# hyye/lio-mapping

Measured on AMD Instinct MI355X. Metric: sliding-window solves/sec, 64-line 130k-pt scans, window=15 (opt_window=5), higher is better.
Workload: dtype f64 (solve) / f32 (features); 1 GPU; HDL-64E outdoor_test_config_64, S_outdoor ray-cast scans, window_size=15 opt_window_size=5, one SolveOptimization per step, clouds resident in HBM; n_lidar_residuals=78236, local_map_points=76752, surf_stack_points=19386, parallelism=1 window

## Files before the change

### include/lio_c.h

```cpp
#ifndef LIO_C_H_
#define LIO_C_H_

#include <stddef.h>
#include <stdint.h>

#ifdef __cplusplus
extern "C" {
#endif

#define LIO_OK 0
#define LIO_ERR_ARG (-1)
#define LIO_ERR_STATE (-2)
#define LIO_ERR_DEVICE (-3)
#define LIO_ERR_CAPACITY (-4)

typedef struct {
  float q[4];
  float p[3];
} lio_transform_f;

const char *lio_backend(void);

typedef struct {
  double scan_period;
// ... 153 lines not shown
  int point_distance_factor;
  int prior_factor;
  int marginalization_factor;
  int enable_deskew;
  int cutoff_deskew;
  int keep_features;
  double acc_n, gyr_n, acc_w, gyr_w, g_norm;
  int max_num_iterations;
  double max_solver_time;
  int extrinsic_stage;
  int init_window_factor;
  int device_solve;
  int inline_marg;
  int stream_sync;
  int resident_moments;
} lio_est_config;

typedef struct {
  int iterations;
  int successful_steps;
  int termination;
  int n_lidar_residuals;
  int n_local_map;
  int laser_odom_iterations;
  int turn_off;
  int convergence_flag;
  int marginalized;
  double cost_pim_before, cost_ppp_before, cost_marg_before;
  double initial_cost, final_cost;
  double cost_trace[32];
// ... 100 lines not shown
```

### lio-mapping_amd/csrc/capi.hip

```cpp
#include <cstring>
#include <new>

#include "../../include/lio_c.h"
#include "../../include/lio_test_hooks.h"
#include "../../include/lio_ext.h"
#include "../../include/lio_full_cloud.h"
#include "../../include/lio_odom_batch.h"
#include "../../include/lio_frontend_batch.h"
#include "../../include/lio_map_batch.h"
#include "est_batch.h"
#include "seg_sort.h"
#include "estimator.h"
#include "rccl_comm.h"
#include "host_init.h"
#include "kf_batch.h"
#include <mutex>
#include <thread>
#include <atomic>
#include <algorithm>

#include "mapping.h"
#include "odometry.h"
#include "pointproc.h"

// ... 560 lines not shown
struct Scratch {
  hipStream_t s = nullptr;
  DBuf<float4> a, b, c;
  VoxelGridDev vox;
  KnnGrid grid;
  DBuf<uint8_t> valid;
  DBuf<float4> coef, abs_coef;
  DBuf<float> score, tf;
  DBuf<int32_t> idx;
  DBuf<float> sqd, nbr;
  DBuf<float> bounds;
  DBuf<double> gn_partials, gn_sums;
  DBuf<OdomState> gn_state;
  DBuf<KfDesc> gn_kd;
  DBuf<float> gn_rows;
};
static Scratch &scratch() {
  static thread_local Scratch sc;
  if (!sc.s) {
    int nd = 0;
    LIO_HIP(hipGetDeviceCount(&nd));
    if (nd <= 0) throw DeviceError("no HIP device: the product has no CPU path");
    LIO_HIP(hipStreamCreate(&sc.s));
  }
  return sc;
}

int lio_voxel_grid(const float *xyzi, size_t n, float leaf, float *out, size_t *n_out) {
  if ((!xyzi && n) || !out || !n_out || !(leaf > 0)) return LIO_ERR_ARG;
  return guarded([&] {
// ... 218 lines not shown
    host_cloud_bounds(map, n_map, mn, mx);
    sc.grid.build(sc.a.p, n_map, mn, mx, knn_cell_edge(mm), sc.s);
    FeatArgs fa{};
    fa.nframes = 1; fa.max_M = M; fa.min_match_sq_dis = mm; fa.min_plane_dis = mp;
    fa.fr[0].stack = sc.b.p; fa.fr[0].M = M; fa.fr[0].slot_off = 0; fa.fr[0].tf_index = 0;
    launch_odom_round(fa, 0, 0, 0, sc.gn_state.p, sc.grid.sorted(), sc.grid.cells(), sc.grid.desc(), sc.valid.p, sc.coef.p, sc.score.p, sc.gn_partials.p, sc.s,
                      nullptr, HostSignal(), lpq);
    if (nb) LIO_HIP(hipMemcpyAsync(partials_out, sc.gn_partials.p, size_t(nb) * 28 * sizeof(double), hipMemcpyDeviceToHost, sc.s));
    LIO_HIP(hipMemcpyAsync(state_out, sc.gn_state.p, sizeof(OdomState), hipMemcpyDeviceToHost, sc.s));
    LIO_HIP(hipStreamSynchronize(sc.s));
    *nb_out = nb;
    return LIO_OK;
  });
}

int lio_calculate_features(const float *map, size_t n_map, const float *stack, size_t m, const lio_transform_f *T, float mm, float mp,
                           uint8_t *valid, float *coeff, float *score) {
  if ((!map && n_map) || (!stack && m) || !T || !valid || !coeff || !score || !(mm > 0)) return LIO_ERR_ARG;
  return guarded([&] {
    Scratch &sc = scratch();
    sc.a.reserve(std::max<size_t>(n_map, 1)); sc.b.reserve(std::max<size_t>(m, 1));
    sc.valid.reserve(std::max<size_t>(m, 1)); sc.coef.reserve(std::max<size_t>(m, 1)); sc.score.reserve(std::max<size_t>(m, 1)); sc.tf.reserve(8);
    if (n_map) LIO_HIP(hipMemcpyAsync(sc.a.p, map, n_map * sizeof(float4), hipMemcpyHostToDevice, sc.s));
    if (m) LIO_HIP(hipMemcpyAsync(sc.b.p, stack, m * sizeof(float4), hipMemcpyHostToDevice, sc.s));
    float tf[8] = {T->q[0], T->q[1], T->q[2], T->q[3], T->p[0], T->p[1], T->p[2], 0.f};
    LIO_HIP(hipMemcpyAsync(sc.tf.p, tf, sizeof(tf), hipMemcpyHostToDevice, sc.s));
    float mn[3], mx[3];
    host_cloud_bounds(map, n_map, mn, mx);
    sc.grid.build(sc.a.p, n_map, mn, mx, knn_cell_edge(mm), sc.s);
    FeatArgs fa{};
// ... 87 lines not shown
  if (!h) return nullptr;
  EstConfig &e = h->cfg;
  e.W = c->window_size; e.Wo = c->opt_window_size;
  e.corner_filter_size = c->corner_filter_size; e.surf_filter_size = c->surf_filter_size;
  e.min_match_sq_dis = c->min_match_sq_dis; e.min_plane_dis = c->min_plane_dis;
  e.transform_lb = toT(c->transform_lb);
  e.opt_extrinsic = c->opt_extrinsic; e.imu_factor = c->imu_factor; e.point_distance_factor = c->point_distance_factor;
  e.prior_factor = c->prior_factor; e.marginalization_factor = c->marginalization_factor;
  e.enable_deskew = c->enable_deskew; e.cutoff_deskew = c->cutoff_deskew; e.keep_features = c->keep_features;
  e.pim.acc_n = c->acc_n; e.pim.gyr_n = c->gyr_n; e.pim.acc_w = c->acc_w; e.pim.gyr_w = c->gyr_w; e.pim.g_norm = c->g_norm;
  e.max_num_iterations = c->max_num_iterations; e.max_solver_time = c->max_solver_time; e.extrinsic_stage = c->extrinsic_stage;
  e.init_window_factor = c->init_window_factor > 0 ? c->init_window_factor : 1;
  e.device_solve = c->device_solve != 0; e.inline_marg = c->inline_marg != 0;
  e.stream_sync = c->stream_sync != 0;
  e.resident_moments = (c->resident_moments >= 1 && c->resident_moments <= 3) ? c->resident_moments : 0;
  h->map_cfg.corner_filter_size = c->corner_filter_size; h->map_cfg.surf_filter_size = c->surf_filter_size;
  h->map_cfg.min_match_sq_dis = c->min_match_sq_dis; h->map_cfg.min_plane_dis = c->min_plane_dis; h->map_cfg.num_max_iterations = 10;
  h->map_cfg.map_builder = 0; h->map_cfg.enable_4d = 1; h->map_cfg.skip_count = 2;
  int rc = guarded([&] {
    h->e.reset(new Estimator(e));
    if (e.device_solve) {
      h->solo.reset(new EstimatorBatch({h->e.get()}));
      EstimatorBatch *b = h->solo.get();
      h->e->solve_hook_ = [b](lio_solve_report *rep) { b->Solve(rep); return b->window_ok(0); };
    }
    return LIO_OK;
  });
  if (rc != LIO_OK) { delete h; return nullptr; }
  return h;
}
// ... 599 lines not shown
```

### lio-mapping_amd/csrc/cloud_device.h

```cpp
#pragma once
#include <hip/hip_runtime.h>

#include <cfloat>
#include <climits>

#include "cloud_kernels.h"
#include "hmath.h"

#if defined(__HIPCC__)
namespace lio {

__device__ inline bool finite3(const float4 &p) { return isfinite(p.x) && isfinite(p.y) && isfinite(p.z); }
__device__ inline bool finite3(const Vec3<float> &p) { return isfinite(p.x) && isfinite(p.y) && isfinite(p.z); }


template <bool NORMALISE_CONJ>
__device__ __forceinline__ float4 to_end_point(float4 p, float s, const Quat<float> &qe, const Vec3<float> &te) {
  p.x -= s * te.x; p.y -= s * te.y; p.z -= s * te.z;
  Quat<float> qid;
  Quat<float> qs = slerp(qid, s, qe, FLT_EPSILON);
  Quat<float> qc = conj(qs);
  if (NORMALISE_CONJ) qc = normalized(qc);
  Vec3<float> v = rotate(qc, Vec3<float>(p.x, p.y, p.z));
  v = rotate(qe, v);
// ... 206 lines not shown
template <int K>
__device__ __forceinline__ void knn_insert(unsigned long long key, int j, unsigned long long (&bk)[K], int (&bj)[K]) {
  if (key < bk[K - 1]) {
    bk[K - 1] = key; bj[K - 1] = j;
#pragma unroll
    for (int k = K - 1; k > 0; --k) {
      const bool sw = bk[k - 1] > bk[k];
      const unsigned long long tk = sw ? bk[k - 1] : bk[k];
      const int tj = sw ? bj[k - 1] : bj[k];
      bk[k - 1] = sw ? bk[k] : bk[k - 1];
      bj[k - 1] = sw ? bj[k] : bj[k - 1];
      bk[k] = tk; bj[k] = tj;
    }
  }
}
template <int K, int LPQ>
__device__ inline void knn_scan_group(const Vec3<float> &q, bool active, int sub, const float4 *__restrict__ map,
                                      const int *__restrict__ cells, const GridDesc &g, float (&bd)[K], int (&bi)[K], int (&bj)[K]) {
  unsigned long long bk[K];
#pragma unroll
  for (int k = 0; k < K; ++k) { bk[k] = knn_key(INFINITY, INT_MAX); bj[k] = 0; }
  int cx, cy, cz;
  cell_of(q.x, q.y, q.z, g, cx, cy, cz);
  if (!finite3(q) || cx < 0 || cy < 0 || cz < 0 || cx >= g.dims[0] || cy >= g.dims[1] || cz >= g.dims[2]) active = false;
  if (active) {
    const int x0 = max(cx - 1, 0), x1 = min(cx + 1, g.dims[0] - 1);
    if constexpr (LPQ <= 2) {
      const float uy = q.y * g.inv_cell, uz = q.z * g.inv_cell;
      const float fy = uy - floorf(uy), fz = uz - floorf(uz);
      const float cell = 1.0f / g.inv_cell;
      const float ey_lo = fmaxf(fy - 1e-3f, 0.f) * cell, ey_hi = fmaxf(1.0f - fy - 1e-3f, 0.f) * cell;
      const float ez_lo = fmaxf(fz - 1e-3f, 0.f) * cell, ez_hi = fmaxf(1.0f - fz - 1e-3f, 0.f) * cell;
      auto walk = [&](int j) {
// ... 27 lines not shown
          if (qq == 1) { s1 = a; c2 = c1 + len; }
          if (qq == 2) { s2 = a; c3 = c2 + len; }
          if (qq == 3) { s3 = a; T = c3 + len; }
        }
        for (int f = 0; f < T; ++f) {
          int j = s0 + f * LPQ;
          j = f >= c1 ? s1 + (f - c1) * LPQ : j;
          j = f >= c2 ? s2 + (f - c2) * LPQ : j;
          j = f >= c3 ? s3 + (f - c3) * LPQ : j;
          walk(j);
        }
      }
    } else {
      int rs[9], pre[10];
      pre[0] = 0;
#pragma unroll
      for (int r = 0; r < 9; ++r) {
        const int z = cz + r / 3 - 1, y = cy + r % 3 - 1;
        const bool in = z >= 0 && z < g.dims[2] && y >= 0 && y < g.dims[1];
        const int row = g.dims[0] * (y + g.dims[1] * z);
        const int a = in ? cells[row + x0] : 0, b = in ? cells[row + x1 + 1] : 0;
        rs[r] = a;
        pre[r + 1] = b - a;
      }
#pragma unroll
      for (int r = 0; r < 9; ++r) pre[r + 1] = pre[r] + max(pre[r + 1], 0);
      const int T = pre[9];
      for (int base = sub; base < T; base += LPQ * KNN_BATCH) {
        float4 p[KNN_BATCH];
        int jj[KNN_BATCH];
#pragma unroll
        for (int b = 0; b < KNN_BATCH; ++b) {
          const int f = base + b * LPQ;
          int j = f + rs[0];
#pragma unroll
          for (int r = 1; r < 9; ++r) j = f >= pre[r] ? f - pre[r] + rs[r] : j;
          jj[b] = f < T ? j : -1;
          p[b] = f < T ? map[j] : make_float4(0, 0, 0, 0);
        }
#pragma unroll
        for (int b = 0; b < KNN_BATCH; ++b) {
          if (jj[b] < 0) continue;
          float ddx = p[b].x - q.x, ddy = p[b].y - q.y, ddz = p[b].z - q.z;
          float d = ddx * ddx;
          d += ddy * ddy;
          d += ddz * ddz;
          knn_insert<K>(knn_key(d, __float_as_int(p[b].w)), jj[b], bk, bj);
        }
      }
    }
  }
#pragma unroll
  for (int m = 1; m < LPQ; m <<= 1) {
    unsigned long long ok[K]; int oj[K];
#pragma unroll
    for (int k = 0; k < K; ++k) {
      const unsigned int lo = __shfl_xor(static_cast<unsigned int>(bk[k]), m, 64), hi = __shfl_xor(static_cast<unsigned int>(bk[k] >> 32), m, 64);
      ok[k] = (static_cast<unsigned long long>(hi) << 32) | lo;
      oj[k] = __shfl_xor(bj[k], m, 64);
    }
#pragma unroll
    for (int c = 0; c < K; ++c) knn_insert<K>(ok[c], oj[c], bk, bj);
  }
#pragma unroll
  for (int k = 0; k < K; ++k) { bd[k] = __uint_as_float(static_cast<unsigned int>(bk[k] >> 32)); bi[k] = int(static_cast<unsigned int>(bk[k])); }
}

struct FeatScalars { float min_match_sq_dis, min_plane_dis; int mapping_mode; float fixed_pz[3]; };
__device__ __forceinline__ FeatScalars feat_scalars(const FeatArgs &a) {
  return FeatScalars{a.min_match_sq_dis, a.min_plane_dis, a.mapping_mode, {a.fixed_pz[0], a.fixed_pz[1], a.fixed_pz[2]}};
}
struct FeatResult { bool owner; uint8_t ok; float4 c; float sc; float4 abs; float4 po; int slot; };
template <bool MAPPING>
__device__ __forceinline__ FeatResult features_fit(const FeatScalars &a, int slot, const Quat<float> &q, const Vec3<float> &t, const float4 &po,
                                                   const Vec3<float> &sel, float bd4, int bi4, const int (&bj)[5], const float4 *__restrict__ map) {
  FeatResult res;
  res.owner = true; res.ok = 0; res.c = make_float4(0, 0, 0, 0); res.sc = 0; res.abs = make_float4(0, 0, 0, 0); res.po = po; res.slot = slot;
  uint8_t ok = 0;
  float4 c = make_float4(0, 0, 0, 0);
  float sc = 0;
// ... 184 lines not shown
  if (!isfinite(t.x)) t.x = 0;
  if (!isfinite(t.y)) t.y = 0;
  if (!isfinite(t.z)) t.z = 0;
  st->T[0] = q.x; st->T[1] = q.y; st->T[2] = q.z; st->T[3] = q.w; st->T[4] = t.x; st->T[5] = t.y; st->T[6] = t.z;
  Quat<float> d = R0 * conj(q);
  float ang = 2.f * atan2f(norm(d.vec()), fabsf(d.w));
  float delta_r = float(double(ang) * 180.0 / M_PI);
  double dt0 = double(X[3] * 100), dt1 = double(X[4] * 100), dt2 = double(X[5] * 100);
  float delta_t = float(sqrt(dt0 * dt0 + dt1 * dt1 + dt2 * dt2));
  st->iters = iter + 1;
  if (double(delta_r) < 0.05 && double(delta_t) < 0.05) st->converged = 1;
}


#define ODOM_ROUND_THREADS 256
template <int LPQ, int THREADS = ODOM_ROUND_THREADS>
__device__ __forceinline__ double odom_round_block(const FeatScalars fs, FeatFrame fr, const Quat<float> q, const Vec3<float> t, const float4 *__restrict__ map,
                                                   const int *__restrict__ cells, const GridDesc &g, uint8_t *__restrict__ valid, float4 *__restrict__ coef,
                                                   float *__restrict__ score, int base_slot, int round, int keep, int block) {
  constexpr int QPB = THREADS / LPQ;
  static_assert(QPB <= 64, "the fit phase is one wave");
  __shared__ int s_bj[QPB][5];
  __shared__ float s_bd4[QPB];
  __shared__ int s_bi4[QPB];
  const int M = fr.M;
  fr.slot_off = base_slot + (keep ? round * M : 0);
  {
    const int ql = threadIdx.x / LPQ, sub = threadIdx.x % LPQ;
    const int i = block * QPB + ql;
    const bool active = i < M;
    const float4 po = active ? fr.stack[i] : make_float4(0, 0, 0, 0);
    const Vec3<float> r = rotate(q, Vec3<float>(po.x, po.y, po.z));
    const Vec3<float> sel(r.x + t.x, r.y + t.y, r.z + t.z);
    float bd[5]; int bi[5], bj[5];
    knn_scan_group<5, LPQ>(sel, active, sub, map, cells, g, bd, bi, bj);
    if (sub == 0) {
#pragma unroll
      for (int k = 0; k < 5; ++k) s_bj[ql][k] = bj[k];
      s_bd4[ql] = bd[4]; s_bi4[ql] = bi[4];
    }
  }
  __syncthreads();
  double v = 0;
  if (threadIdx.x < 64) {
    const int ql = threadIdx.x;
    double acc[28];
#pragma unroll
    for (int k = 0; k < 28; ++k) acc[k] = 0;
    const int i = block * QPB + ql;
    if (ql < QPB && i < M) {
      const float4 po = fr.stack[i];
      const Vec3<float> r = rotate(q, Vec3<float>(po.x, po.y, po.z));
      const Vec3<float> sel(r.x + t.x, r.y + t.y, r.z + t.z);
      int bj[5];
// ... 81 lines not shown
```

### lio-mapping_amd/csrc/cloud_kernels.h

```cpp
#pragma once
#include <cmath>
#include <cstdint>

#include "dev.h"
#include "hmath.h"

namespace lio {

struct VoxParams {
  float mn[3], mx[3];
  int minb[3], divb[3];
  int overflow;
  int n_valid;
};

struct Affine3f { float m[12]; };

#define LIO_MAX_FRAMES 32

struct ConcatSeg { const float4 *src; int n; int dst_off; int set_intensity; float intensity; Affine3f tf; int identity; };
struct ConcatArgs { ConcatSeg seg[LIO_MAX_FRAMES]; int nseg; int total; };
void launch_transform_concat(const ConcatArgs &a, float4 *dst, hipStream_t s);

void launch_deskew_to_end(float4 *pts, int n, const float q[4], const float p[3], float time_factor, hipStream_t s, bool keep_intensity = false);
// ... 115 lines not shown
  int kz;
  int nsel;
};
inline OdomState odom_state_at(const Rigid<float> &T) {
  OdomState st{};
  st.T[0] = T.rot.x; st.T[1] = T.rot.y; st.T[2] = T.rot.z; st.T[3] = T.rot.w;
  st.T[4] = T.pos.x; st.T[5] = T.pos.y; st.T[6] = T.pos.z;
  return st;
}
inline void point_on_z_axis(const Rigid<float> &T, float pz[3]) {
  const Vec3<float> z = rotate(T.rot, Vec3<float>(0.f, 0.f, 10.f));
  pz[0] = z.x + T.pos.x; pz[1] = z.y + T.pos.y; pz[2] = z.z + T.pos.z;
}
int odom_rows_blocks(int nslots);
int odom_round_blocks(int M, int lpq);
void launch_odom_round(const FeatArgs &a, int base_slot, int round, int keep, OdomState *st, const float4 *map_sorted, const int *cells, const GridDesc &g,
                       uint8_t *valid, float4 *coef, float *score, double *partials, hipStream_t s, OdomState *mail = nullptr,
                       const HostSignal &sig = HostSignal(), int lpq = 8);

void launch_gn_rows_map(const float4 *stack, int m, const uint8_t *valid, const float4 *coef, const OdomState *st, int b_from_coef, uint8_t *ok_out,
                        float *rows_out, hipStream_t s);
void launch_gn_fold(const double *partials, int nblocks, int wide, double *sums_out, hipStream_t s);
void launch_gn_step(const double *sums, OdomState *st, int iter, int min_rows, int left_update, hipStream_t s);

struct KfDesc {
  int slot_off, Mc, Ms;
  int map;
  int nb;
  int part_off;
  float pz[3];
};
struct KfMapDesc {
  const float4 *corner_sorted; const int *corner_cells; GridDesc corner_grid;
// ... 34 lines not shown
```

### lio-mapping_amd/csrc/cloud_kernels.hip

```cpp
#include <cstring>
#include <hip/hip_runtime.h>
#include <rocprim/rocprim.hpp>

#include <cfloat>
#include <climits>

#include "cloud_kernels.h"
#include "cloud_device.h"

namespace lio {

__global__ void k_transform_concat(ConcatArgs a, float4 *__restrict__ dst) {
  int gid = blockIdx.x * blockDim.x + threadIdx.x;
  if (gid >= a.total) return;
  int sidx = 0;
  for (int k = 1; k < a.nseg; ++k)
    if (gid >= a.seg[k].dst_off) sidx = k;
  const ConcatSeg &sg = a.seg[sidx];
  int local = gid - sg.dst_off;
  float4 p = sg.src[local];
  float4 o;
  if (sg.identity) {
    o = p;
  } else {
// ... 487 lines not shown
  __syncthreads();
  if (threadIdx.x < 28) {
    double v = 0;
    for (int w = 0; w < ODOM_ROW_THREADS / 64; ++w) v += sm[w][threadIdx.x];
    partials[block_x * 28 + threadIdx.x] = v;
  }
}

__device__ __forceinline__ void odom_update_body(const double *__restrict__ partials, int nblocks, OdomState *st, int iter, int min_rows,
                                                 int left_update) {
  __shared__ double ssum[28];
  reduce_partials28(partials, nblocks, ssum);
  odom_update_from_sums(ssum, st, iter, min_rows, left_update);
}

template <int LPQ>
__global__ void __launch_bounds__(ODOM_ROUND_THREADS) k_odom_round(FeatArgs a, const OdomState *__restrict__ st, const float4 *__restrict__ map,
                                                                  const int *__restrict__ cells, GridDesc g, uint8_t *__restrict__ valid,
                                                                  float4 *__restrict__ coef, float *__restrict__ score, double *__restrict__ partials,
                                                                  int base_slot, int round, int keep) {
  if (st->converged) return;
  const float *tp = st->T;
  const Quat<float> q(tp[3], tp[0], tp[1], tp[2]);
  const Vec3<float> t(tp[4], tp[5], tp[6]);
  const double v = odom_round_block<LPQ>(feat_scalars(a), a.fr[0], q, t, map, cells, g, valid, coef, score, base_slot, round, keep, int(blockIdx.x));
  if (threadIdx.x < 28) partials[size_t(blockIdx.x) * 28 + threadIdx.x] = v;
}

__global__ void __launch_bounds__(1024) k_odom_update_wide(const double *__restrict__ partials, int nblocks, OdomState *st, int iter, int min_rows,
                                                           int left_update, OdomState *mail, HostSignal sig) {
  odom_update_wide_block(partials, nblocks, st, iter, min_rows, left_update, mail, sig);
}
__global__ void __launch_bounds__(256) k_solve_setup(SolveSetup a, float *__restrict__ d_transforms, OdomState *__restrict__ d_odom, uint8_t *__restrict__ valid,
                                                     size_t n_valid) {
  clear_valid_block(valid, n_valid);
  if (blockIdx.x == 0) {
    for (int k = threadIdx.x; k < a.ntf * 8; k += 256) d_transforms[k] = a.tf[k >> 3][k & 7];
    if (a.set_odom) odom_state_init(d_odom, a.odom_T, false);
  }
}
void launch_solve_setup(const SolveSetup &a, float *d_transforms, OdomState *d_odom, uint8_t *valid, size_t n_valid, hipStream_t s) {
  const int nb = std::max(1, cdiv((long long)n_valid, 256 * 16));
  hipLaunchKernelGGL(k_solve_setup, dim3(nb), dim3(256), 0, s, a, d_transforms, d_odom, valid, n_valid);
  LIO_HIP(hipGetLastError());
}

int odom_round_blocks(int M, int lpq) { return std::max(1, cdiv((long long)M * lpq, ODOM_ROUND_THREADS)); }
void launch_odom_round(const FeatArgs &a, int base_slot, int round, int keep, OdomState *st, const float4 *map_sorted, const int *cells, const GridDesc &g,
                       uint8_t *valid, float4 *coef, float *score, double *partials, hipStream_t s, OdomState *mail, const HostSignal &sig, int lpq) {
  const int M = a.fr[0].M;
  if (M <= 0) return;
  const int nb = odom_round_blocks(M, lpq);
  if (lpq == 4)
    hipLaunchKernelGGL(k_odom_round<4>, dim3(nb), dim3(ODOM_ROUND_THREADS), 0, s, a, st, map_sorted, cells, g, valid, coef, score, partials, base_slot, round, keep);
  else
    hipLaunchKernelGGL(k_odom_round<8>, dim3(nb), dim3(ODOM_ROUND_THREADS), 0, s, a, st, map_sorted, cells, g, valid, coef, score, partials, base_slot, round, keep);
  hipLaunchKernelGGL(k_odom_update_wide, dim3(1), dim3(1024), 0, s, partials, nb, st, round, 0, 0, mail, sig);
  LIO_HIP(hipGetLastError());
}

__global__ void __launch_bounds__(256) k_gn_rows_map(const float4 *__restrict__ stack, int m, const uint8_t *__restrict__ valid, const float4 *__restrict__ coef,
                                                     const OdomState *__restrict__ st, int b_from_coef, uint8_t *__restrict__ ok_out,
                                                     float *__restrict__ rows_out) {
  const int i = blockIdx.x * blockDim.x + threadIdx.x;
  if (i >= m) return;
  Quat<float> q(st->T[3], st->T[0], st->T[1], st->T[2]);
  Vec3<float> t(st->T[4], st->T[5], st->T[6]);
  Mat3<float> Rm = toRot(q);
  Mat3<float> Rinv = toRot(qinverse(q));
  float a[6] = {0, 0, 0, 0, 0, 0}, bb = 0;
  const bool ok = valid[i] != 0;
  if (ok) odom_row_form(stack[i], coef[i], q, t, Rm, Rinv, b_from_coef, a, bb);
// ... 147 lines not shown
```

### lio-mapping_amd/csrc/estimator.h

```cpp
#pragma once
#include <climits>
#include <condition_variable>
#include <exception>
#include <functional>
#include <memory>
#include <mutex>
#include <thread>
#include <vector>

#include "../../include/lio_c.h"
#include "cloud_kernels.h"
#include "host_init.h"
#include "host_solver.h"
#include "batch_kernels.h"
#include "resident_moments.h"
#include "solve_step.h"

namespace lio {

typedef Rigid<float> Rigidf;
typedef Rigid<double> Rigidd;

struct EstConfig {
  int W = 15, Wo = 5;
  float corner_filter_size = 0.2f, surf_filter_size = 0.4f, min_match_sq_dis = 1.0f, min_plane_dis = 0.2f;
  Rigidf transform_lb;
  bool opt_extrinsic = false, imu_factor = true, point_distance_factor = false, prior_factor = false, marginalization_factor = true,
       enable_deskew = true, cutoff_deskew = false, keep_features = false;
  PimNoise pim;
  int max_num_iterations = 10;
  double max_solver_time = 0.10;
  int extrinsic_stage = 2;
  int init_window_factor = 3;
  bool device_solve = false, inline_marg = false, stream_sync = false;
  int resident_moments = 0;
};

struct DeviceCloud {
  DBuf<float4> buf;
  size_t n = 0;
  uint64_t id = 0;
  DeviceCloud() = default;
  DeviceCloud(DeviceCloud &&o) noexcept : buf(std::move(o.buf)), n(o.n), id(o.id) { o.n = 0; o.id = 0; }
  DeviceCloud &operator=(DeviceCloud &&o) noexcept {
    if (this != &o) { buf = std::move(o.buf); n = o.n; id = o.id; o.n = 0; o.id = 0; }
    return *this;
  }
};

struct StampedPose { double time; Rigidf T; };
// ... 249 lines not shown
  std::vector<size_t> size_surf_stack_;
  std::vector<StampedPose> imu_stamped_;
  DeviceCloud local_, local_filtered_, scratch_cloud_, upload_;
  VoxelGridDev vox_;
  KnnGrid grid_;
  DBuf<uint8_t> f_valid_;
  DBuf<float4> f_coef_;
  DBuf<float> f_score_;
  std::vector<int> slot_off_, nslots_;
  size_t total_slots_ = 0;
  EstimatorBatch *feat_batch_ = nullptr;
  int feat_batch_w_ = -1;
  DBuf<float> d_transforms_;
  DBuf<OdomState> d_odom_;
  DBuf<double> d_odom_partials_, d_moment_partials_, d_moment_out_;
  HostBuf<double> h_moment_out_;
  HostBuf<OdomState> h_odom_;
  HostBuf<unsigned> h_signal_;
  unsigned signal_seq_[2] = {0, 0};
  bool host_signal_ = true;
  int device_id_ = 0;
  HostSignal moment_signal_{};
  bool frames_dirty_ = true;
  std::unique_ptr<HostState> snap_;
  std::vector<DeviceCloud> snap_stacks_;
  bool map_refresh_ = false;
  std::vector<OptSlot> opt_ring_;
  long frame_seq_ = 0;
  std::shared_ptr<DeviceCloud> corner_last_;
  std::vector<std::shared_ptr<DeviceCloud>> corner_pool_;
// ... 16 lines not shown
```

### lio-mapping_amd/csrc/estimator.hip

```cpp
#include "estimator.h"
#include "est_batch.h"
#include "mapping.h"
#include "marg_kernels.h"
#include "rccl_comm.h"

#include <atomic>
#include <cfloat>
#include <climits>
#include <cstring>

namespace lio {

static const bool g_debug_timing = std::getenv("LIO_DEBUG_TIMING") != nullptr;

static V3d R2ypr(const M3d &R) {
  V3d n(R(0, 0), R(1, 0), R(2, 0)), o(R(0, 1), R(1, 1), R(2, 1)), a(R(0, 2), R(1, 2), R(2, 2));
  double y = atan2(n.y, n.x);
  double p = atan2(-n.z, n.x * cos(y) + n.y * sin(y));
  double r = atan2(a.x * sin(y) - a.y * cos(y), -o.x * sin(y) + o.y * cos(y));
  return V3d(y, p, r) / M_PI * 180.0;
}
static M3d ypr2R(const V3d &ypr) {
  double y = ypr.x / 180.0 * M_PI, p = ypr.y / 180.0 * M_PI, r = ypr.z / 180.0 * M_PI;
  M3d Rz, Ry, Rx;
// ... 632 lines not shown
    timers_.end(th, sf);
    if (sf != stream_) LIO_HIP(hipEventRecord(ev_join_, sf));
  }
  laser_odom_iters_ = 0; laser_odom_kz_ = 0;
  if (cfg_.imu_factor) {
    OdomState st{};
    bool have_state = false;
    std::memcpy(st.T, pl.tf[W_], 8 * sizeof(float));
    const int M = int(stacks_[W_].n);
    const bool mail = host_signal_ && !timers_.on;
    HostSignal sig{};
    if (M > 0) {
      const int lpq = 8;
      const int nb = odom_round_blocks(M, lpq);
      d_odom_partials_.reserve(size_t(nb) * 28);
      FeatArgs fo{};
      fo.min_match_sq_dis = cfg_.min_match_sq_dis; fo.min_plane_dis = cfg_.min_plane_dis;
      fo.nframes = 1; fo.max_M = M;
      fo.fr[0].stack = stacks_[W_].buf.p; fo.fr[0].M = M; fo.fr[0].tf_index = 0; fo.fr[0].slot_off = slot_off_[W_];
      const int chunk_end[4] = {3, 5, 7, 10};
      int chunk = 0;
      for (int iter = 0; iter < 10; ++iter) {
        if (iter == chunk_end[chunk]) {
          if (mail) {
            wait_host_signal(sig, stream_);
          } else {
            LIO_HIP(hipMemcpyAsync(h_odom_.p, d_odom_.p, sizeof(st), hipMemcpyDeviceToHost, stream_));
            LIO_HIP(hipStreamSynchronize(stream_));
          }
          st = *h_odom_.p;
          if (st.converged) { have_state = true; break; }
          ++chunk;
        }
        if (mail) { sig.flag = h_signal_.p + 128; sig.seq = ++signal_seq_[1]; }
        const double ns = keep_mult > 1 ? double(iter + 1) * M : double(M);
        int t1h = timers_.begin(KT_ODOM_FEATURES, 16.0 * (double(M) + double(local_filtered_.n)) + 72.0 * M + 33.0 * ns, stream_);
        launch_odom_round(fo, slot_off_[W_], iter, keep_mult > 1 ? 1 : 0, d_odom_.p, grid_.sorted(), grid_.cells(), grid_.desc(), f_valid_.p, f_coef_.p,
                          f_score_.p, d_odom_partials_.p, stream_, mail ? h_odom_.p : nullptr, sig, lpq);
        timers_.end(t1h, stream_);
      }
    }
    LIO_HIP(hipStreamWaitEvent(stream_, ev_join_, 0));
    if (!have_state) {
      if (sig.flag) {
        wait_host_signal(sig, stream_);
      } else {
        LIO_HIP(hipMemcpyAsync(h_odom_.p, d_odom_.p, sizeof(st), hipMemcpyDeviceToHost, stream_));
        LIO_HIP(hipStreamSynchronize(stream_));
      }
      st = *h_odom_.p;
      timers_.resolve();
    }
    ApplyOdomState(st);
// ... 544 lines not shown
```

### lio-mapping_amd/lio_amd/capi.py

```python
from __future__ import annotations

import ctypes as C
import os

import numpy as np

_HERE = os.path.dirname(os.path.abspath(__file__))
HIP_LIB_PATH = os.environ.get("LIO_HIP_LIB") or os.path.join(os.path.dirname(_HERE), "csrc", "liblio_hip.so")

c_double_p = C.POINTER(C.c_double)
c_float_p = C.POINTER(C.c_float)
c_int32_p = C.POINTER(C.c_int32)
c_uint8_p = C.POINTER(C.c_uint8)
c_uint16_p = C.POINTER(C.c_uint16)


class TransformF(C.Structure):
    _fields_ = [("q", C.c_float * 4), ("p", C.c_float * 3)]

    @staticmethod
    def make(q_xyzw, p):
        t = TransformF()
        for i in range(4):
            t.q[i] = float(q_xyzw[i])
# ... 51 lines not shown
        ("cutoff_deskew", C.c_int),
        ("keep_features", C.c_int),
        ("acc_n", C.c_double),
        ("gyr_n", C.c_double),
        ("acc_w", C.c_double),
        ("gyr_w", C.c_double),
        ("g_norm", C.c_double),
        ("max_num_iterations", C.c_int),
        ("max_solver_time", C.c_double),
        ("extrinsic_stage", C.c_int),
        ("init_window_factor", C.c_int),
        ("device_solve", C.c_int),
        ("inline_marg", C.c_int),
        ("stream_sync", C.c_int),
        ("resident_moments", C.c_int),
    ]


class SolveReport(C.Structure):
    _fields_ = [
        ("iterations", C.c_int),
        ("successful_steps", C.c_int),
        ("termination", C.c_int),
        ("n_lidar_residuals", C.c_int),
        ("n_local_map", C.c_int),
        ("laser_odom_iterations", C.c_int),
        ("turn_off", C.c_int),
        ("convergence_flag", C.c_int),
        ("marginalized", C.c_int),
        ("cost_pim_before", C.c_double),
# ... 162 lines not shown
    "lio_gn_fold": (C.c_int, [c_double_p, C.c_int, C.c_int, c_double_p]),
    "lio_gn_step": (C.c_int, [C.c_int, c_double_p, C.c_void_p, C.c_int, C.c_int, C.c_int, C.c_void_p]),
    "lio_gn_round": (C.c_int, [c_float_p, C.c_size_t, c_float_p, C.c_size_t, C.POINTER(TransformF), C.c_float, C.c_float, C.c_int, c_int32_p,
                               c_double_p, C.c_void_p]),
}
GN_STATE = np.dtype([("T", np.float32, 8), ("converged", np.int32), ("iters", np.int32), ("degenerate", np.int32), ("kz", np.int32),
                     ("nsel", np.int32)])
_EXT_SIGS = {
    "lio_est_map": (C.c_void_p, [C.c_void_p]),
    "lio_est_set_map_refresh": (C.c_int, [C.c_void_p, C.c_int]),
    "lio_est_refresh_map": (C.c_int, [C.c_void_p]),
    "lio_map_get_surround": (C.c_size_t, [C.c_void_p, C.c_float, c_float_p]),
    "lio_est_get_last_map_refresh": (C.c_int, [C.c_void_p, C.POINTER(C.c_int), C.POINTER(TransformF), C.POINTER(C.c_int), C.POINTER(C.c_uint32),
                                               C.POINTER(C.c_int), C.POINTER(C.c_size_t), c_float_p, C.POINTER(C.c_size_t), c_float_p]),
}
_FULL_SIGS = {
    "lio_odom_full_to_end": (C.c_int, [C.c_void_p, c_float_p, C.c_size_t, c_float_p]),
    "lio_map_set_full_cloud": (C.c_int, [C.c_void_p, c_float_p, C.c_size_t]),
    "lio_map_get_full_cloud": (C.c_size_t, [C.c_void_p, c_float_p]),
    "lio_est_set_full_cloud": (C.c_int, [C.c_void_p, C.c_int]),
    "lio_est_get_full_stack": (C.c_size_t, [C.c_void_p, C.c_int, c_float_p, C.POINTER(C.c_int)]),
    "lio_est_get_registered_full": (C.c_int, [C.c_void_p, C.c_int, C.POINTER(TransformF), C.POINTER(C.c_size_t), c_float_p]),
    "lio_est_get_full_transform_es": (C.c_int, [C.c_void_p, C.c_int, C.POINTER(TransformF)]),
    "lio_deskew_to_end": (C.c_int, [c_float_p, C.c_size_t, C.POINTER(TransformF), C.c_float, C.c_int, c_float_p]),
}
FULL_MAP_FRAME, FULL_SENSOR_RAW, FULL_SENSOR_END = 1, 2, 3
_c_float_pp, _c_size_p = C.POINTER(c_float_p), C.POINTER(C.c_size_t)
_ODOM_BATCH_SIGS = {
    "lio_odom_process_batch": (C.c_int, [C.POINTER(C.c_void_p), C.c_int, _c_float_pp, _c_size_p, _c_float_pp, _c_size_p, _c_float_pp, _c_size_p,
                                         _c_float_pp, _c_size_p, C.POINTER(TransformF), C.POINTER(TransformF), c_int32_p, c_int32_p]),
# ... 49 lines not shown
        for name, (res, args) in _TEST_SIGS.items():
            fn = getattr(self.dll, name, None)
            if fn is None:
                self.missing.append(name)
                continue
            fn.restype = res
            fn.argtypes = args
        self.backend = self.dll.lio_backend().decode()
        self.has_ext = self.backend.startswith("hip")
        if self.has_ext:
            for name, (res, args) in (list(_EXT_SIGS.items()) + list(_FULL_SIGS.items()) + list(_ODOM_BATCH_SIGS.items()) + list(_FRONTEND_SIGS.items())
                                      + list(_MAP_BATCH_SIGS.items())):
                fn = getattr(self.dll, name)
                fn.restype = res
                fn.argtypes = args

    def deskew_to_end(self, xyzi, T_es: TransformF, time_factor=10.0, keep_intensity=False):
        c = _f32(xyzi).reshape(-1, 4)
        out = np.zeros_like(c)
        _chk(self.dll.lio_deskew_to_end(_fp(c), c.shape[0], C.byref(T_es), time_factor, 1 if keep_intensity else 0, _fp(out)), "lio_deskew_to_end")
        return out

    @staticmethod
    def _laser_frames(transforms, pims):
        n = len(transforms)
        T = (TransformF * n)(*[TransformF.make(q, p) for q, p in transforms])
        P = (C.c_void_p * n)(*[(p.h if p is not None else None) for p in pims])
        return n, T, P

    def imu_estimate_extrinsic_rotation(self, transforms, pims, T_lb):
# ... 146 lines not shown
        _chk(self.dll.lio_gn_step(int(family), s_.ctypes.data_as(c_double_p), si.ctypes.data, int(iter), int(min_rows), int(left_update),
                                  so.ctypes.data), "lio_gn_step")
        return so[0]

    def gn_round(self, map_xyzi, stack_xyzi, T: TransformF, lanes_per_query, min_match_sq_dis=1.0, min_plane_dis=0.2):
        m_ = _f32(map_xyzi).reshape(-1, 4)
        s_ = _f32(stack_xyzi).reshape(-1, 4)
        m = s_.shape[0]
        nb = np.zeros(1, dtype=np.int32)
        partials = np.zeros((max(1, -(-m * int(lanes_per_query) // 256)), 28), dtype=np.float64)
        so = np.zeros(1, dtype=GN_STATE)
        _chk(self.dll.lio_gn_round(_fp(m_), m_.shape[0], _fp(s_), m, C.byref(T), float(min_match_sq_dis), float(min_plane_dis),
                                   int(lanes_per_query), nb.ctypes.data_as(c_int32_p), partials.ctypes.data_as(c_double_p), so.ctypes.data),
             "lio_gn_round")
        return partials[: int(nb[0])].copy(), so[0]

    def calculate_features(self, map_xyzi, stack_xyzi, T: TransformF, min_match_sq_dis=1.0, min_plane_dis=0.2):
        m_ = _f32(map_xyzi).reshape(-1, 4)
        s_ = _f32(stack_xyzi).reshape(-1, 4)
        valid = np.zeros(s_.shape[0], dtype=np.uint8)
        coeff = np.zeros((s_.shape[0], 4), dtype=np.float32)
        score = np.zeros(s_.shape[0], dtype=np.float32)
        _chk(
            self.dll.lio_calculate_features(
                _fp(m_), m_.shape[0], _fp(s_), s_.shape[0], C.byref(T), min_match_sq_dis, min_plane_dis, valid.ctypes.data_as(c_uint8_p), _fp(coeff), _fp(score)
            ),
            "lio_calculate_features",
        )
        return valid, coeff, score

# ... 824 lines not shown
```

Baseline: 2116 solves/s.

## Bound later-round KNN search with previous round's neighbour list

Odometry Gauss-Newton rounds now save each query's 5 nearest neighbours. Later rounds use those points' distances, under the new pose, as an upper bound on the search. The grid walk then skips neighbouring cell rows and x-extents that lie entirely beyond the bound, and skips heap inserts above it. This is on by default (round_search=0), and it adds per-query neighbour-list writes and reads plus some bound computation in exchange for less map-point scanning.

```diff
diff --git a/include/lio_c.h b/include/lio_c.h
--- a/include/lio_c.h
+++ b/include/lio_c.h
@@ -191,6 +191,7 @@
   int inline_marg;
   int stream_sync;
   int resident_moments;
+  int round_search;
 } lio_est_config;
 
 typedef struct {
diff --git a/include/lio_round_search.h b/include/lio_round_search.h
--- /dev/null
+++ b/include/lio_round_search.h
@@ -0,0 +1,17 @@
+#ifndef LIO_ROUND_SEARCH_H
+#define LIO_ROUND_SEARCH_H
+
+#include "lio_c.h"
+
+#ifdef __cplusplus
+extern "C" {
+#endif
+
+int lio_gn_rounds(const float *map_xyzi, size_t n_map, const float *stack_xyzi, size_t m, const lio_transform_f *T, int n_rounds,
+                  float min_match_sq_dis, float min_plane_dis, int lanes_per_query, int search, int32_t *nb_out, uint8_t *valid_out,
+                  float *coeff_out, double *partials_out, int32_t *idx_out, int32_t *n_bounded_out);
+
+#ifdef __cplusplus
+}
+#endif
+#endif
diff --git a/lio-mapping_amd/csrc/capi.hip b/lio-mapping_amd/csrc/capi.hip
--- a/lio-mapping_amd/csrc/capi.hip
+++ b/lio-mapping_amd/csrc/capi.hip
@@ -8,6 +8,7 @@
 #include "../../include/lio_odom_batch.h"
 #include "../../include/lio_frontend_batch.h"
 #include "../../include/lio_map_batch.h"
+#include "../../include/lio_round_search.h"
 #include "est_batch.h"
 #include "seg_sort.h"
 #include "estimator.h"
@@ -598,6 +599,7 @@
   DBuf<OdomState> gn_state;
   DBuf<KfDesc> gn_kd;
   DBuf<float> gn_rows;
+  DBuf<int> gn_nn, gn_idx, gn_count;
 };
 static Scratch &scratch() {
   static thread_local Scratch sc;
@@ -846,6 +848,49 @@
   });
 }
 
+int lio_gn_rounds(const float *map, size_t n_map, const float *stack, size_t m, const lio_transform_f *T, int n_rounds, float mm, float mp, int lpq,
+                  int search, int32_t *nb_out, uint8_t *valid_out, float *coeff_out, double *partials_out, int32_t *idx_out, int32_t *n_bounded_out) {
+  if ((!map && n_map) || !stack || !m || !T || !nb_out || !valid_out || !coeff_out || !partials_out || !idx_out || !n_bounded_out) return LIO_ERR_ARG;
+  if (!(lpq == 4 || lpq == 8) || !(search == 0 || search == 1) || n_rounds < 1 || n_rounds > 16) return LIO_ERR_ARG;
+  if (!(mm > 0) || !std::isfinite(mm) || !(mp > 0) || !std::isfinite(mp)) return LIO_ERR_ARG;
+  for (int r = 0; r < n_rounds; ++r)
+    if (!finite_T(T + r)) return LIO_ERR_ARG;
+  if (m > size_t(INT_MAX) / 8 || n_map > size_t(INT_MAX)) return LIO_ERR_CAPACITY;
+  return guarded([&] {
+    Scratch &sc = scratch();
+    const int M = int(m), nb = odom_round_blocks(M, lpq);
+    sc.a.reserve(std::max<size_t>(n_map, 1)); sc.b.reserve(m);
+    sc.valid.reserve(m); sc.coef.reserve(m); sc.score.reserve(m);
+    sc.gn_partials.reserve(size_t(nb) * 28); sc.gn_state.reserve(1);
+    sc.gn_nn.reserve(m * 5); sc.gn_idx.reserve(m * 5); sc.gn_count.reserve(1);
+    if (n_map) LIO_HIP(hipMemcpyAsync(sc.a.p, map, n_map * sizeof(float4), hipMemcpyHostToDevice, sc.s));
+    LIO_HIP(hipMemcpyAsync(sc.b.p, stack, m * sizeof(float4), hipMemcpyHostToDevice, sc.s));
+    float mn[3], mx[3];
+    host_cloud_bounds(map, n_map, mn, mx);
+    sc.grid.build(sc.a.p, n_map, mn, mx, knn_cell_edge(mm), sc.s);
+    FeatArgs fa{};
+    fa.nframes = 1; fa.max_M = M; fa.min_match_sq_dis = mm; fa.min_plane_dis = mp;
+    fa.fr[0].stack = sc.b.p; fa.fr[0].M = M; fa.fr[0].slot_off = 0; fa.fr[0].tf_index = 0;
+    RoundList rl;
+    rl.nn = search == 0 ? sc.gn_nn.p : nullptr; rl.idx_out = sc.gn_idx.p; rl.n_bounded = sc.gn_count.p;
+    for (int r = 0; r < n_rounds; ++r) {
+      const OdomState st = odom_state_at(toT(T[r]));
+      LIO_HIP(hipMemcpyAsync(sc.gn_state.p, &st, sizeof(st), hipMemcpyHostToDevice, sc.s));
+      LIO_HIP(hipMemsetAsync(sc.gn_count.p, 0, sizeof(int), sc.s));
+      launch_odom_round(fa, 0, r, 0, sc.gn_state.p, sc.grid.sorted(), sc.grid.cells(), sc.grid.desc(), sc.valid.p, sc.coef.p, sc.score.p, sc.gn_partials.p,
+                        sc.s, nullptr, HostSignal(), lpq, rl, search == 0 ? (r == 0 ? 1 : 2) : 0);
+      LIO_HIP(hipMemcpyAsync(valid_out + size_t(r) * m, sc.valid.p, m, hipMemcpyDeviceToHost, sc.s));
+      LIO_HIP(hipMemcpyAsync(coeff_out + size_t(r) * m * 4, sc.coef.p, m * sizeof(float4), hipMemcpyDeviceToHost, sc.s));
+      LIO_HIP(hipMemcpyAsync(partials_out + size_t(r) * nb * 28, sc.gn_partials.p, size_t(nb) * 28 * sizeof(double), hipMemcpyDeviceToHost, sc.s));
+      LIO_HIP(hipMemcpyAsync(idx_out + size_t(r) * m * 5, sc.gn_idx.p, m * 5 * sizeof(int), hipMemcpyDeviceToHost, sc.s));
+      LIO_HIP(hipMemcpyAsync(n_bounded_out + r, sc.gn_count.p, sizeof(int), hipMemcpyDeviceToHost, sc.s));
+      LIO_HIP(hipStreamSynchronize(sc.s));
+    }
+    *nb_out = nb;
+    return LIO_OK;
+  });
+}
+
 int lio_calculate_features(const float *map, size_t n_map, const float *stack, size_t m, const lio_transform_f *T, float mm, float mp,
                            uint8_t *valid, float *coeff, float *score) {
   if ((!map && n_map) || (!stack && m) || !T || !valid || !coeff || !score || !(mm > 0)) return LIO_ERR_ARG;
@@ -963,6 +1008,7 @@
   e.device_solve = c->device_solve != 0; e.inline_marg = c->inline_marg != 0;
   e.stream_sync = c->stream_sync != 0;
   e.resident_moments = (c->resident_moments >= 1 && c->resident_moments <= 3) ? c->resident_moments : 0;
+  e.round_search = c->round_search == 1 ? 1 : 0;
   h->map_cfg.corner_filter_size = c->corner_filter_size; h->map_cfg.surf_filter_size = c->surf_filter_size;
   h->map_cfg.min_match_sq_dis = c->min_match_sq_dis; h->map_cfg.min_plane_dis = c->min_plane_dis; h->map_cfg.num_max_iterations = 10;
   h->map_cfg.map_builder = 0; h->map_cfg.enable_4d = 1; h->map_cfg.skip_count = 2;
diff --git a/lio-mapping_amd/csrc/cloud_device.h b/lio-mapping_amd/csrc/cloud_device.h
--- a/lio-mapping_amd/csrc/cloud_device.h
+++ b/lio-mapping_amd/csrc/cloud_device.h
@@ -244,9 +244,11 @@
     }
   }
 }
-template <int K, int LPQ>
+template <int K, int LPQ, bool BOUND = false>
 __device__ inline void knn_scan_group(const Vec3<float> &q, bool active, int sub, const float4 *__restrict__ map,
-                                      const int *__restrict__ cells, const GridDesc &g, float (&bd)[K], int (&bi)[K], int (&bj)[K]) {
+                                      const int *__restrict__ cells, const GridDesc &g, float (&bd)[K], int (&bi)[K], int (&bj)[K],
+                                      unsigned long long B = 0) {
+  static_assert(!BOUND || LPQ > 2, "the bounded walk is the multi-lane form");
   unsigned long long bk[K];
 #pragma unroll
   for (int k = 0; k < K; ++k) { bk[k] = knn_key(INFINITY, INT_MAX); bj[k] = 0; }
@@ -304,12 +306,30 @@
     } else {
       int rs[9], pre[10];
       pre[0] = 0;
+      float D = 0.f, ex_lo = 0.f, ex_hi = 0.f, ey_lo = 0.f, ey_hi = 0.f, ez_lo = 0.f, ez_hi = 0.f;
+      if constexpr (BOUND) {
+        D = __uint_as_float(static_cast<unsigned int>(B >> 32));
+        const float ux = q.x * g.inv_cell, uy = q.y * g.inv_cell, uz = q.z * g.inv_cell;
+        const float fx = ux - floorf(ux), fy = uy - floorf(uy), fz = uz - floorf(uz);
+        const float cell = 1.0f / g.inv_cell;
+        ex_lo = fmaxf(fx - 1e-3f, 0.f) * cell; ex_hi = fmaxf(1.0f - fx - 1e-3f, 0.f) * cell;
+        ey_lo = fmaxf(fy - 1e-3f, 0.f) * cell; ey_hi = fmaxf(1.0f - fy - 1e-3f, 0.f) * cell;
+        ez_lo = fmaxf(fz - 1e-3f, 0.f) * cell; ez_hi = fmaxf(1.0f - fz - 1e-3f, 0.f) * cell;
+      }
 #pragma unroll
       for (int r = 0; r < 9; ++r) {
         const int z = cz + r / 3 - 1, y = cy + r % 3 - 1;
-        const bool in = z >= 0 && z < g.dims[2] && y >= 0 && y < g.dims[1];
+        bool in = z >= 0 && z < g.dims[2] && y >= 0 && y < g.dims[1];
         const int row = g.dims[0] * (y + g.dims[1] * z);
-        const int a = in ? cells[row + x0] : 0, b = in ? cells[row + x1 + 1] : 0;
+        int xa = x0, xb = x1;
+        if constexpr (BOUND) {
+          const float ey = r % 3 == 0 ? ey_lo : (r % 3 == 2 ? ey_hi : 0.f), ez = r / 3 == 0 ? ez_lo : (r / 3 == 2 ? ez_hi : 0.f);
+          const float e2 = ey * ey + ez * ez;
+          in = in && !(e2 > D);
+          xa = ex_lo * ex_lo + e2 > D ? cx : x0;
+          xb = ex_hi * ex_hi + e2 > D ? cx : x1;
+        }
+        const int a = in ? cells[row + xa] : 0, b = in ? cells[row + xb + 1] : 0;
         rs[r] = a;
         pre[r + 1] = b - a;
       }
@@ -335,7 +355,12 @@
           float d = ddx * ddx;
           d += ddy * ddy;
           d += ddz * ddz;
-          knn_insert<K>(knn_key(d, __float_as_int(p[b].w)), jj[b], bk, bj);
+          const unsigned long long key = knn_key(d, __float_as_int(p[b].w));
+          if constexpr (BOUND) {
+            if (key <= B) knn_insert<K>(key, jj[b], bk, bj);
+          } else {
+            knn_insert<K>(key, jj[b], bk, bj);
+          }
         }
       }
     }
@@ -354,6 +379,44 @@
   }
 #pragma unroll
   for (int k = 0; k < K; ++k) { bd[k] = __uint_as_float(static_cast<unsigned int>(bk[k] >> 32)); bi[k] = int(static_cast<unsigned int>(bk[k])); }
+}
+
+template <int LPQ>
+__device__ __forceinline__ unsigned long long knn_prev_bound(const Vec3<float> &q, bool active, int sub, const int *prev,
+                                                             const float4 *__restrict__ map, const GridDesc &g, bool &bounded) {
+  constexpr unsigned long long BROKEN = ~0ull;
+  int cx, cy, cz;
+  const bool inside = cell_of(q.x, q.y, q.z, g, cx, cy, cz);
+  const bool ok = active && finite3(q) && inside && prev[4] >= 0;
+  unsigned long long key = 0;
+#pragma unroll
+  for (int kk = 0; kk < (5 + LPQ - 1) / LPQ; ++kk) {
+    const int k = sub + kk * LPQ;
+    if (ok && k < 5) {
+      const int j = prev[k];
+      unsigned long long kj = BROKEN;
+      if (unsigned(j) < unsigned(g.n_points)) {
+        const float4 pc = map[j];
+        int px, py, pz;
+        cell_of(pc.x, pc.y, pc.z, g, px, py, pz);
+        px = min(max(px, 0), g.dims[0] - 1); py = min(max(py, 0), g.dims[1] - 1); pz = min(max(pz, 0), g.dims[2] - 1);
+        float ddx = pc.x - q.x, ddy = pc.y - q.y, ddz = pc.z - q.z;
+        float d = ddx * ddx;
+        d += ddy * ddy;
+        d += ddz * ddz;
+        if (abs(px - cx) <= 1 && abs(py - cy) <= 1 && abs(pz - cz) <= 1) kj = knn_key(d, __float_as_int(pc.w));
+      }
+      key = kj > key ? kj : key;
+    }
+  }
+#pragma unroll
+  for (int m = 1; m < LPQ; m <<= 1) {
+    const unsigned int lo = __shfl_xor(static_cast<unsigned int>(key), m, 64), hi = __shfl_xor(static_cast<unsigned int>(key >> 32), m, 64);
+    const unsigned long long o = (static_cast<unsigned long long>(hi) << 32) | lo;
+    key = o > key ? o : key;
+  }
+  bounded = ok && key != BROKEN;
+  return bounded ? key : knn_key(INFINITY, INT_MAX);
 }
 
 struct FeatScalars { float min_match_sq_dis, min_plane_dis; int mapping_mode; float fixed_pz[3]; };
@@ -568,10 +631,11 @@
 
 
 #define ODOM_ROUND_THREADS 256
-template <int LPQ, int THREADS = ODOM_ROUND_THREADS>
+template <int LPQ, int THREADS = ODOM_ROUND_THREADS, int LIST = 0, bool STATS = false>
 __device__ __forceinline__ double odom_round_block(const FeatScalars fs, FeatFrame fr, const Quat<float> q, const Vec3<float> t, const float4 *__restrict__ map,
                                                    const int *__restrict__ cells, const GridDesc &g, uint8_t *__restrict__ valid, float4 *__restrict__ coef,
-                                                   float *__restrict__ score, int base_slot, int round, int keep, int block) {
+                                                   float *__restrict__ score, int base_slot, int round, int keep, int block,
+                                                   const RoundList rl = RoundList()) {
   constexpr int QPB = THREADS / LPQ;
   static_assert(QPB <= 64, "the fit phase is one wave");
   __shared__ int s_bj[QPB][5];
@@ -587,11 +651,29 @@
     const Vec3<float> r = rotate(q, Vec3<float>(po.x, po.y, po.z));
     const Vec3<float> sel(r.x + t.x, r.y + t.y, r.z + t.z);
     float bd[5]; int bi[5], bj[5];
-    knn_scan_group<5, LPQ>(sel, active, sub, map, cells, g, bd, bi, bj);
+    if constexpr (LIST == 2) {
+      bool bounded;
+      const unsigned long long B = knn_prev_bound<LPQ>(sel, active, sub, rl.nn + size_t(i) * 5, map, g, bounded);
+      if constexpr (STATS)
+        if (bounded && sub == 0) atomicAdd(rl.n_bounded, 1);
+      knn_scan_group<5, LPQ, true>(sel, active, sub, map, cells, g, bd, bi, bj, B);
+    } else {
+      knn_scan_group<5, LPQ>(sel, active, sub, map, cells, g, bd, bi, bj);
+    }
     if (sub == 0) {
 #pragma unroll
       for (int k = 0; k < 5; ++k) s_bj[ql][k] = bj[k];
       s_bd4[ql] = bd[4]; s_bi4[ql] = bi[4];
+      if constexpr (LIST != 0)
+        if (active) {
+#pragma unroll
+          for (int k = 0; k < 5; ++k) rl.nn[size_t(i) * 5 + k] = (k == 4 && bi[4] == INT_MAX) ? -1 : bj[k];
+        }
+      if constexpr (STATS)
+        if (active) {
+#pragma unroll
+          for (int k = 0; k < 5; ++k) rl.idx_out[size_t(i) * 5 + k] = bi[k];
+        }
     }
   }
   __syncthreads();
diff --git a/lio-mapping_amd/csrc/cloud_kernels.h b/lio-mapping_amd/csrc/cloud_kernels.h
--- a/lio-mapping_amd/csrc/cloud_kernels.h
+++ b/lio-mapping_amd/csrc/cloud_kernels.h
@@ -153,9 +153,10 @@
 }
 int odom_rows_blocks(int nslots);
 int odom_round_blocks(int M, int lpq);
+struct RoundList { int *nn = nullptr; int *idx_out = nullptr; int *n_bounded = nullptr; };
 void launch_odom_round(const FeatArgs &a, int base_slot, int round, int keep, OdomState *st, const float4 *map_sorted, const int *cells, const GridDesc &g,
                        uint8_t *valid, float4 *coef, float *score, double *partials, hipStream_t s, OdomState *mail = nullptr,
-                       const HostSignal &sig = HostSignal(), int lpq = 8);
+                       const HostSignal &sig = HostSignal(), int lpq = 8, const RoundList &rl = RoundList(), int list_mode = 0);
 
 void launch_gn_rows_map(const float4 *stack, int m, const uint8_t *valid, const float4 *coef, const OdomState *st, int b_from_coef, uint8_t *ok_out,
                         float *rows_out, hipStream_t s);
diff --git a/lio-mapping_amd/csrc/cloud_kernels.hip b/lio-mapping_amd/csrc/cloud_kernels.hip
--- a/lio-mapping_amd/csrc/cloud_kernels.hip
+++ b/lio-mapping_amd/csrc/cloud_kernels.hip
@@ -1,4 +1,5 @@
 #include <cstring>
+#include <stdexcept>
 #include <hip/hip_runtime.h>
 #include <rocprim/rocprim.hpp>
 
@@ -525,16 +526,17 @@
   odom_update_from_sums(ssum, st, iter, min_rows, left_update);
 }
 
-template <int LPQ>
+template <int LPQ, int LIST = 0, bool STATS = false>
 __global__ void __launch_bounds__(ODOM_ROUND_THREADS) k_odom_round(FeatArgs a, const OdomState *__restrict__ st, const float4 *__restrict__ map,
                                                                   const int *__restrict__ cells, GridDesc g, uint8_t *__restrict__ valid,
                                                                   float4 *__restrict__ coef, float *__restrict__ score, double *__restrict__ partials,
-                                                                  int base_slot, int round, int keep) {
+                                                                  int base_slot, int round, int keep, RoundList rl) {
   if (st->converged) return;
   const float *tp = st->T;
   const Quat<float> q(tp[3], tp[0], tp[1], tp[2]);
   const Vec3<float> t(tp[4], tp[5], tp[6]);
-  const double v = odom_round_block<LPQ>(feat_scalars(a), a.fr[0], q, t, map, cells, g, valid, coef, score, base_slot, round, keep, int(blockIdx.x));
+  const double v = odom_round_block<LPQ, ODOM_ROUND_THREADS, LIST, STATS>(feat_scalars(a), a.fr[0], q, t, map, cells, g, valid, coef, score, base_slot, round,
+                                                                        keep, int(blockIdx.x), rl);
   if (threadIdx.x < 28) partials[size_t(blockIdx.x) * 28 + threadIdx.x] = v;
 }
 
@@ -557,16 +559,26 @@
 }
 
 int odom_round_blocks(int M, int lpq) { return std::max(1, cdiv((long long)M * lpq, ODOM_ROUND_THREADS)); }
+using OdomRoundKernel = void (*)(FeatArgs, const OdomState *, const float4 *, const int *, GridDesc, uint8_t *, float4 *, float *, double *, int, int, int,
+                                 RoundList);
+template <int LPQ, bool STATS>
+static OdomRoundKernel odom_round_kernel(int list_mode) {
+  return list_mode == 0 ? k_odom_round<LPQ, 0, STATS> : list_mode == 1 ? k_odom_round<LPQ, 1, STATS> : k_odom_round<LPQ, 2, STATS>;
+}
 void launch_odom_round(const FeatArgs &a, int base_slot, int round, int keep, OdomState *st, const float4 *map_sorted, const int *cells, const GridDesc &g,
-                       uint8_t *valid, float4 *coef, float *score, double *partials, hipStream_t s, OdomState *mail, const HostSignal &sig, int lpq) {
+                       uint8_t *valid, float4 *coef, float *score, double *partials, hipStream_t s, OdomState *mail, const HostSignal &sig, int lpq,
+                       const RoundList &rl, int list_mode) {
   const int M = a.fr[0].M;
   if (M <= 0) return;
   const int nb = odom_round_blocks(M, lpq);
-  if (lpq == 4)
-    hipLaunchKernelGGL(k_odom_round<4>, dim3(nb), dim3(ODOM_ROUND_THREADS), 0, s, a, st, map_sorted, cells, g, valid, coef, score, partials, base_slot, round, keep);
-  else
-    hipLaunchKernelGGL(k_odom_round<8>, dim3(nb), dim3(ODOM_ROUND_THREADS), 0, s, a, st, map_sorted, cells, g, valid, coef, score, partials, base_slot, round, keep);
-  hipLaunchKernelGGL(k_odom_update_wide, dim3(1), dim3(1024), 0, s, partials, nb, st, round, 0, 0, mail, sig);
+  const bool stats = rl.idx_out != nullptr;
+  if (list_mode < 0 || list_mode > 2 || (list_mode != 0 && !rl.nn) || (stats != (rl.n_bounded != nullptr)))
+    throw std::invalid_argument("launch_odom_round: neighbour list and mode do not agree");
+  const OdomRoundKernel k = stats ? (lpq == 4 ? odom_round_kernel<4, true>(list_mode) : odom_round_kernel<8, true>(list_mode))
+                                  : (lpq == 4 ? odom_round_kernel<4, false>(list_mode) : odom_round_kernel<8, false>(list_mode));
+  hipLaunchKernelGGL(k, dim3(nb), dim3(ODOM_ROUND_THREADS), 0, s, a, st, map_sorted, cells, g, valid, coef, score, partials, base_slot, round, keep, rl);
+  if (!stats)
+    hipLaunchKernelGGL(k_odom_update_wide, dim3(1), dim3(1024), 0, s, partials, nb, st, round, 0, 0, mail, sig);
   LIO_HIP(hipGetLastError());
 }
 
diff --git a/lio-mapping_amd/csrc/estimator.h b/lio-mapping_amd/csrc/estimator.h
--- a/lio-mapping_amd/csrc/estimator.h
+++ b/lio-mapping_amd/csrc/estimator.h
@@ -34,6 +34,7 @@
   int init_window_factor = 3;
   bool device_solve = false, inline_marg = false, stream_sync = false;
   int resident_moments = 0;
+  int round_search = 0;
 };
 
 struct DeviceCloud {
@@ -313,6 +314,7 @@
   DBuf<float> d_transforms_;
   DBuf<OdomState> d_odom_;
   DBuf<double> d_odom_partials_, d_moment_partials_, d_moment_out_;
+  DBuf<int> d_odom_nn_;
   HostBuf<double> h_moment_out_;
   HostBuf<OdomState> h_odom_;
   HostBuf<unsigned> h_signal_;
diff --git a/lio-mapping_amd/csrc/estimator.hip b/lio-mapping_amd/csrc/estimator.hip
--- a/lio-mapping_amd/csrc/estimator.hip
+++ b/lio-mapping_amd/csrc/estimator.hip
@@ -670,6 +670,9 @@
       const int lpq = 8;
       const int nb = odom_round_blocks(M, lpq);
       d_odom_partials_.reserve(size_t(nb) * 28);
+      const bool bounded = cfg_.round_search == 0;
+      RoundList rl{};
+      if (bounded) { d_odom_nn_.reserve(size_t(M) * 5); rl.nn = d_odom_nn_.p; }
       FeatArgs fo{};
       fo.min_match_sq_dis = cfg_.min_match_sq_dis; fo.min_plane_dis = cfg_.min_plane_dis;
       fo.nframes = 1; fo.max_M = M;
@@ -692,7 +695,7 @@
         const double ns = keep_mult > 1 ? double(iter + 1) * M : double(M);
         int t1h = timers_.begin(KT_ODOM_FEATURES, 16.0 * (double(M) + double(local_filtered_.n)) + 72.0 * M + 33.0 * ns, stream_);
         launch_odom_round(fo, slot_off_[W_], iter, keep_mult > 1 ? 1 : 0, d_odom_.p, grid_.sorted(), grid_.cells(), grid_.desc(), f_valid_.p, f_coef_.p,
-                          f_score_.p, d_odom_partials_.p, stream_, mail ? h_odom_.p : nullptr, sig, lpq);
+                          f_score_.p, d_odom_partials_.p, stream_, mail ? h_odom_.p : nullptr, sig, lpq, rl, bounded ? (iter == 0 ? 1 : 2) : 0);
         timers_.end(t1h, stream_);
       }
     }
diff --git a/lio-mapping_amd/lio_amd/capi.py b/lio-mapping_amd/lio_amd/capi.py
--- a/lio-mapping_amd/lio_amd/capi.py
+++ b/lio-mapping_amd/lio_amd/capi.py
@@ -89,6 +89,7 @@
         ("inline_marg", C.c_int),
         ("stream_sync", C.c_int),
         ("resident_moments", C.c_int),
+        ("round_search", C.c_int),
     ]
 
 
@@ -281,6 +282,10 @@
     "lio_est_get_last_map_refresh": (C.c_int, [C.c_void_p, C.POINTER(C.c_int), C.POINTER(TransformF), C.POINTER(C.c_int), C.POINTER(C.c_uint32),
                                                C.POINTER(C.c_int), C.POINTER(C.c_size_t), c_float_p, C.POINTER(C.c_size_t), c_float_p]),
 }
+_ROUND_SEARCH_SIGS = {
+    "lio_gn_rounds": (C.c_int, [c_float_p, C.c_size_t, c_float_p, C.c_size_t, C.POINTER(TransformF), C.c_int, C.c_float, C.c_float, C.c_int, C.c_int,
+                                c_int32_p, c_uint8_p, c_float_p, c_double_p, c_int32_p, c_int32_p]),
+}
 _FULL_SIGS = {
     "lio_odom_full_to_end": (C.c_int, [C.c_void_p, c_float_p, C.c_size_t, c_float_p]),
     "lio_map_set_full_cloud": (C.c_int, [C.c_void_p, c_float_p, C.c_size_t]),
@@ -360,6 +365,11 @@
                 fn = getattr(self.dll, name)
                 fn.restype = res
                 fn.argtypes = args
+            for name, (res, args) in _ROUND_SEARCH_SIGS.items():
+                fn = getattr(self.dll, name, None)
+                if fn is not None:
+                    fn.restype = res
+                    fn.argtypes = args
 
     def deskew_to_end(self, xyzi, T_es: TransformF, time_factor=10.0, keep_intensity=False):
         c = _f32(xyzi).reshape(-1, 4)
@@ -536,6 +546,25 @@
                                    int(lanes_per_query), nb.ctypes.data_as(c_int32_p), partials.ctypes.data_as(c_double_p), so.ctypes.data),
              "lio_gn_round")
         return partials[: int(nb[0])].copy(), so[0]
+
+    def gn_rounds(self, map_xyzi, stack_xyzi, transforms, lanes_per_query, search, min_match_sq_dis=1.0, min_plane_dis=0.2):
+        m_ = _f32(map_xyzi).reshape(-1, 4)
+        s_ = _f32(stack_xyzi).reshape(-1, 4)
+        m, R = s_.shape[0], len(transforms)
+        nbmax = max(1, -(-m * int(lanes_per_query) // 256))
+        T = (TransformF * R)(*transforms)
+        nb = np.zeros(1, dtype=np.int32)
+        valid = np.zeros((R, m), dtype=np.uint8)
+        coeff = np.zeros((R, m, 4), dtype=np.float32)
+        partials = np.zeros((R, nbmax, 28), dtype=np.float64)
+        idx = np.zeros((R, m, 5), dtype=np.int32)
+        nbd = np.zeros(R, dtype=np.int32)
+        _chk(self.dll.lio_gn_rounds(_fp(m_), m_.shape[0], _fp(s_), m, T, R, float(min_match_sq_dis), float(min_plane_dis), int(lanes_per_query),
+                                    int(search), nb.ctypes.data_as(c_int32_p), valid.ctypes.data_as(c_uint8_p), _fp(coeff),
+                                    partials.ctypes.data_as(c_double_p), idx.ctypes.data_as(c_int32_p), nbd.ctypes.data_as(c_int32_p)),
+             "lio_gn_rounds")
+        assert int(nb[0]) == nbmax
+        return dict(valid=valid, coeff=coeff, partials=partials, idx=idx, n_bounded=nbd)
 
     def calculate_features(self, map_xyzi, stack_xyzi, T: TransformF, min_match_sq_dis=1.0, min_plane_dis=0.2):
         m_ = _f32(map_xyzi).reshape(-1, 4)
diff --git a/profiles/round_search_summary.py b/profiles/round_search_summary.py
--- /dev/null
+++ b/profiles/round_search_summary.py
@@ -0,0 +1,41 @@
+import csv
+import statistics
+import sys
+
+
+def main():
+    path = sys.argv[1]
+    skip = int(sys.argv[2]) if len(sys.argv) > 2 else 24
+    rows = []
+    with open(path, newline="") as fh:
+        for r in csv.DictReader(fh):
+            rows.append((int(r["Start_Timestamp"]), int(r["End_Timestamp"]), r["Kernel_Name"]))
+    rows.sort()
+    solve, rnd = -1, 0
+    search, update = {}, {}
+    for t0, t1, name in rows:
+        if "k_solve_setup" in name:
+            solve, rnd = solve + 1, 0
+        elif "k_odom_round" in name:
+            if solve >= skip:
+                search.setdefault(rnd, []).append((t1 - t0) / 1e3)
+        elif "k_odom_update_wide" in name:
+            if solve >= skip:
+                update.setdefault(rnd, []).append((t1 - t0) / 1e3)
+            rnd += 1
+    print(f"{path}: {solve + 1} solves, the first {skip} left out")
+    print("| round | launches | k_odom_round mean / median us | k_odom_update_wide mean / median us |")
+    print("|---|---|---|---|")
+    for k in sorted(search):
+        s, u = search[k], update.get(k, [0.0])
+        print(f"| {k} | {len(s)} | {statistics.mean(s):.2f} / {statistics.median(s):.2f} | {statistics.mean(u):.2f} / {statistics.median(u):.2f} |")
+    later = [x for k in search if k >= 1 for x in search[k]]
+    if later:
+        print(f"rounds >= 1: k_odom_round mean {statistics.mean(later):.2f} us, median {statistics.median(later):.2f} us over {len(later)} launches")
+    allu = [x for k in update for x in update[k]]
+    if allu:
+        print(f"k_odom_update_wide: mean {statistics.mean(allu):.2f} us, median {statistics.median(allu):.2f} us over {len(allu)} launches")
+
+
+if __name__ == "__main__":
+    main()
```

Result: no change. 2159 solves/s (median of 4 runs) (+2.0%).
